# rnajena/dynamont

Measured on AMD Instinct MI355X. Metric: signal samples resquiggled/sec, higher is better.
Workload: dtype f64

## Files before the change

dynamont_amd/_native.py:

```python
from __future__ import annotations

import ctypes as C
import os
import subprocess

HERE = os.path.dirname(os.path.abspath(__file__))
CSRC = os.path.join(HERE, "csrc")
LIB_PATH = os.environ.get("DYN_LIB_PATH") or os.path.join(HERE, "libdynamont_mi.so")
SOURCES = ["dynamont_mi.cpp", "buffers.cpp", "launch.cpp", "session.cpp", "async_engine.cpp", "pore_model.cpp", "csv_format.cpp", "csv_sink.cpp", "vbz_decode.cpp", "bam_reader.cpp", "rccl_comm.cpp", "model_format.cpp",
           "nt_kernels.hip", "pool_stats.hip", "wide_band.hip", "event_stats.hip", "rescale.hip"]
HEADERS = ["engine.hpp", "engine_internal.hpp", "zstd_dl.hpp", "vbz_decode.hpp", "nt_kernels.hpp", "pore_model.hpp", "dp_math.hpp", "dp_math_strict.hpp", "dp_cell.hpp", "strict_exp_table.inc", os.path.join("..", "..", "include", "dynamont_mi.h")]

DYN_DEVICE_HOST_ONLY = -2
DYN_CSV_EVENT_STATS = 0x1
DYN_OK, DYN_ERR_INVALID_ARGUMENT, DYN_ERR_RUNTIME, DYN_ERR_DEVICE, DYN_ERR_OUT_OF_MEMORY = range(5)

c_double_p = C.POINTER(C.c_double)
c_float_p = C.POINTER(C.c_float)
c_u64_p = C.POINTER(C.c_uint64)
c_i32_p = C.POINTER(C.c_int32)
c_u8_p = C.POINTER(C.c_uint8)


class DynInfo(C.Structure):
    _fields_ = [("abi_version", C.c_int32), ("pore", C.c_int32), ("rna", C.c_int32), ("kmer_size", C.c_int32),
                ("alphabet_size", C.c_int32), ("device", C.c_int32), ("num_kmers", C.c_uint64),
                ("half_band", C.c_uint64), ("log_m1", C.c_double), ("log_e1", C.c_double), ("log_e2", C.c_double),
                ("max_half_band", C.c_uint64)]


class DynAlignOut(C.Structure):
    _fields_ = [("Z", c_double_p), ("status", c_i32_p), ("bad_char", C.c_void_p), ("seg_offsets", c_u64_p),
                ("n_segments", c_u64_p), ("sequence_positions", c_u64_p), ("signal_positions", c_u64_p),
                ("probabilities", c_double_p), ("states", c_u8_p), ("capacity", C.c_uint64)]


class DynEventOut(C.Structure):
    _fields_ = [("mean", c_double_p), ("stdev", c_double_p), ("median", c_double_p), ("capacity", C.c_uint64)]


class DynRescaleOut(C.Structure):
    _fields_ = [("shift", c_double_p), ("scale", c_double_p), ("iters_applied", c_i32_p), ("n", C.c_uint64)]


class DynTrainOut(C.Structure):
    _fields_ = [("Z", c_double_p), ("status", c_i32_p), ("bad_char", C.c_void_p), ("transitions", c_double_p),
                ("em_offsets", c_u64_p), ("em_count", c_u64_p), ("em_code", c_i32_p), ("em_mean", c_double_p),
                ("em_stdev", c_double_p), ("em_weight", c_double_p), ("em_sum", c_double_p),
                ("em_sumsq", c_double_p), ("trans_counts", c_double_p), ("capacity", C.c_uint64)]


class DynJobBatch(C.Structure):
    _fields_ = [("n", C.c_uint64),
                ("names", C.c_void_p), ("name_off", C.POINTER(C.c_uint64)), ("names_bytes", C.c_uint64),
                ("signal_ids", C.c_void_p), ("signal_id_off", C.POINTER(C.c_uint64)), ("signal_ids_bytes", C.c_uint64),
                ("signal_uuid", C.c_void_p), ("signal_uuid_ok", C.c_void_p),
                ("seqs", C.c_void_p), ("seq_off", C.POINTER(C.c_uint64)), ("seqs_bytes", C.c_uint64),
                ("shift", C.POINTER(C.c_double)), ("scale", C.POINTER(C.c_double)),
                ("start", C.POINTER(C.c_int64)), ("end", C.POINTER(C.c_int64)),
                ("n_files", C.c_uint64), ("files", C.c_void_p), ("file_off", C.POINTER(C.c_uint64)), ("files_bytes", C.c_uint64),
                ("file_id", C.POINTER(C.c_uint32)), ("bases", C.POINTER(C.c_uint32))]


class DynTiming(C.Structure):
    _fields_ = [("ms_total", C.c_double), ("ms_dp", C.c_double), ("ms_backward", C.c_double), ("ms_forward", C.c_double),
                ("ms_trace", C.c_double), ("wave_wait_share", C.c_double), ("wave_occupancy", C.c_double),
                ("cells", C.c_uint64), ("samples", C.c_uint64), ("reads_ok", C.c_uint64),
                ("launches", C.c_uint32), ("lp_inplace", C.c_uint32), ("pool_pages", C.c_uint32),
                ("page_rows", C.c_uint32), ("n_static", C.c_uint32), ("n_waves", C.c_uint32),
                ("reads_strict", C.c_uint32), ("reserved", C.c_uint32),
                ("ms_backward_strict", C.c_double), ("ms_forward_strict", C.c_double), ("cert_fallbacks", C.c_uint64),
                ("cert_rows", C.c_uint64), ("launch_share", C.c_double)]


class DynSessionStats(C.Structure):
    _fields_ = [("sessions", C.c_uint64), ("tickets", C.c_uint64), ("reads", C.c_uint64), ("cells", C.c_uint64), ("ms", C.c_double),
                ("wave_cycles_busy", C.c_uint64), ("wave_cycles_idle", C.c_uint64), ("wave_cycles_life", C.c_uint64),
                ("waves", C.c_uint64), ("aborted", C.c_uint64), ("republished", C.c_uint64)]


SIGNATURES = {
    "dyn_pore_from_string": (C.c_int, [C.c_char_p, C.POINTER(C.c_int), C.c_char_p, C.c_uint64]),
    "dyn_aligner_create": (C.c_int, [C.c_char_p, C.c_int, C.c_char_p, C.c_int, C.c_uint64, C.c_int,
                                     C.POINTER(C.c_void_p), C.c_char_p, C.c_uint64]),
    "dyn_aligner_destroy": (None, [C.c_void_p]),
    "dyn_release_cached_memory": (None, []),
    "dyn_aligner_set_model": (C.c_int, [C.c_void_p, c_double_p]),
    "dyn_format_model": (C.c_uint64, [C.c_char_p, C.c_int, c_double_p, c_double_p, C.c_uint64, C.c_char_p, C.c_uint64]),
    "dyn_aligner_info": (C.c_int, [C.c_void_p, C.POINTER(DynInfo)]),
    "dyn_aligner_model": (C.c_int, [C.c_void_p, c_double_p]),
    "dyn_aligner_session_stats": (C.c_int, [C.c_void_p, C.POINTER(DynSessionStats)]),
    "dyn_aligner_session_page_wait": (C.c_int, [C.c_void_p, c_u64_p]),
    "dyn_aligner_session_idle_split": (C.c_int, [C.c_void_p, C.POINTER(C.c_uint64)]),
    "dyn_aligner_set_session_mode": (C.c_int, [C.c_void_p, C.c_int, C.c_int]),
    "dyn_aligner_set_mem_budget": (C.c_int, [C.c_void_p, C.c_uint64]),
    "dyn_aligner_set_strict": (C.c_int, [C.c_void_p, C.c_int]),
    "dyn_aligner_set_train_zcheck": (C.c_int, [C.c_void_p, C.c_int]),
    "dyn_aligner_set_event_stats": (C.c_int, [C.c_void_p, C.c_int]),
    "dyn_aligner_set_rescale": (C.c_int, [C.c_void_p, C.c_int]),
    "dyn_tie_rows": (C.c_uint32, [C.c_void_p, c_i32_p, C.c_uint64, C.c_uint64]),
    "dyn_aligner_last_error": (C.c_char_p, [C.c_void_p]),
    "dyn_read_strerror": (C.c_int, [C.c_int, C.c_char, C.c_char_p, C.c_uint64]),
    "dyn_segment_capacity": (C.c_uint64, [C.c_void_p, C.c_uint64, c_u64_p]),
    "dyn_validate_batch": (C.c_int, [C.c_void_p, C.c_uint64, c_u64_p, C.c_char_p, c_u64_p, c_i32_p, C.c_void_p,
                                     c_i32_p, C.c_uint64]),
    "dyn_align_batch": (C.c_int, [C.c_void_p, C.c_uint64, c_double_p, c_u64_p, C.c_char_p, c_u64_p, C.c_int,
                                  C.POINTER(DynAlignOut)]),
    "dyn_train_batch": (C.c_int, [C.c_void_p, C.c_uint64, c_double_p, c_u64_p, C.c_char_p, c_u64_p,
                                  C.POINTER(DynTrainOut), c_double_p]),
    "dyn_format_csv_bound": (C.c_uint64, [C.c_void_p, C.c_uint64, C.POINTER(DynAlignOut), C.POINTER(C.c_char_p),
                                          C.POINTER(C.c_char_p)]),
    "dyn_format_csv": (C.c_int, [C.c_void_p, C.c_uint64, C.POINTER(DynAlignOut), C.c_char_p, c_u64_p,
                                 C.POINTER(C.c_char_p), C.POINTER(C.c_char_p), C.POINTER(C.c_int64),
                                 C.POINTER(C.c_int64), C.c_int, C.c_void_p, C.c_uint64, c_u64_p, c_u64_p]),
    "dyn_format_csv_bound_events": (C.c_uint64, [C.c_void_p, C.c_uint64, C.POINTER(DynAlignOut), C.POINTER(DynEventOut),
                                                 C.POINTER(C.c_char_p), C.POINTER(C.c_char_p)]),
    "dyn_format_csv_events": (C.c_int, [C.c_void_p, C.c_uint64, C.POINTER(DynAlignOut), C.POINTER(DynEventOut), C.c_char_p,
                                        c_u64_p, C.POINTER(C.c_char_p), C.POINTER(C.c_char_p), C.POINTER(C.c_int64),
                                        C.POINTER(C.c_int64), C.c_int, C.c_void_p, C.c_uint64, c_u64_p, c_u64_p]),
    "dyn_csv_compact": (C.c_uint64, [C.c_void_p, C.c_uint64, c_u64_p, c_u64_p]),
    "dyn_csv_sink_open": (C.c_int, [C.c_char_p, C.c_char_p, C.c_int, C.c_int, C.POINTER(C.c_void_p), C.c_char_p, C.c_uint64]),
    "dyn_csv_sink_open_part": (C.c_int, [C.c_char_p, C.c_char_p, C.c_int, C.c_int, C.c_int, C.c_int, C.POINTER(C.c_void_p), C.c_char_p, C.c_uint64]),
    "dyn_csv_sink_open_ex": (C.c_int, [C.c_char_p, C.c_char_p, C.c_int, C.c_int, C.c_int, C.c_int, C.c_uint32,
                                       C.POINTER(C.c_void_p), C.c_char_p, C.c_uint64]),
    "dyn_csv_sink_submit": (C.c_int, [C.c_void_p, C.c_void_p, C.c_void_p, C.POINTER(DynAlignOut), C.c_uint64, C.c_char_p, c_u64_p,
                                      C.POINTER(C.c_char_p), C.POINTER(C.c_char_p), C.POINTER(C.c_int64), c_u64_p]),
    "dyn_csv_sink_submit_bases": (C.c_int, [C.c_void_p, C.c_void_p, C.c_void_p, C.POINTER(DynAlignOut), C.c_uint64, C.c_char_p, c_u64_p,
                                            C.POINTER(C.c_char_p), C.POINTER(C.c_char_p), C.POINTER(C.c_int64), c_u64_p, C.POINTER(C.c_uint32)]),
    "dyn_csv_sink_error_line": (C.c_int, [C.c_void_p, C.c_char_p]),
    "dyn_csv_sink_completed": (C.c_uint64, [C.c_void_p]),
    "dyn_csv_sink_wait": (C.c_uint64, [C.c_void_p, C.c_uint64, C.c_int]),
    "dyn_csv_sink_failed": (C.c_int, [C.c_void_p]),
    "dyn_csv_sink_close": (C.c_int, [C.c_void_p, c_u64_p, c_u64_p, c_u64_p, C.c_char_p, C.c_uint64]),
    "dyn_bam_open": (C.c_int, [C.c_char_p, C.c_int, C.c_char_p, C.POINTER(C.c_void_p), C.c_char_p, C.c_uint64]),
    "dyn_bam_next": (C.c_int, [C.c_void_p, C.c_uint64, C.c_uint32, C.c_double, C.c_uint32, C.c_uint32, C.POINTER(DynJobBatch),
                               C.c_char_p, C.c_uint64]),
    "dyn_bam_skipped": (C.c_uint64, [C.c_void_p]),
    "dyn_bam_close": (None, [C.c_void_p]),
    "dyn_batch_create": (C.c_int, [C.c_void_p, C.c_uint64, c_double_p, c_u64_p, C.c_char_p, c_u64_p,
                                   C.POINTER(C.c_void_p)]),
    "dyn_batch_create_raw": (C.c_int, [C.c_void_p, C.c_uint64, C.c_void_p, C.c_int, c_u64_p, c_double_p, c_double_p,
                                       C.c_int, C.c_double, C.c_int, C.c_char_p, c_u64_p, C.POINTER(C.c_void_p)]),
    "dyn_batch_signals": (C.c_int, [C.c_void_p, c_double_p, C.c_uint64]),
    "dyn_batch_destroy": (None, [C.c_void_p]),
    "dyn_batch_align": (C.c_int, [C.c_void_p, C.c_int]),
    "dyn_batch_train": (C.c_int, [C.c_void_p]),
    "dyn_batch_fetch": (C.c_int, [C.c_void_p, C.POINTER(DynAlignOut)]),
    "dyn_batch_fetch_events": (C.c_int, [C.c_void_p, C.POINTER(DynEventOut)]),
    "dyn_batch_fetch_rescale": (C.c_int, [C.c_void_p, C.POINTER(DynRescaleOut)]),
    "dyn_batch_fetch_train": (C.c_int, [C.c_void_p, C.POINTER(DynTrainOut), c_double_p]),
    "dyn_batch_device_results": (C.c_int, [C.c_void_p, C.POINTER(C.c_void_p), c_u64_p, C.POINTER(C.c_void_p)]),
    "dyn_batch_device_pooled": (C.c_int, [C.c_void_p, C.POINTER(C.c_void_p), c_u64_p]),
    "dyn_batch_timing": (C.c_int, [C.c_void_p, C.POINTER(DynTiming)]),
    "dyn_plan_queue": (C.c_int, [C.c_uint64, C.POINTER(C.c_uint32), c_u64_p, C.c_uint64, C.c_uint64, C.POINTER(C.c_uint32),
                                 c_u64_p, c_u64_p]),
    "dyn_session_order": (C.c_int, [C.c_uint64, C.POINTER(C.c_uint32)]),
    "dyn_batch_align_async": (C.c_int, [C.c_void_p, C.c_uint64, c_double_p, c_u64_p, C.c_char_p, c_u64_p, C.c_int,
                                        C.POINTER(DynAlignOut), C.POINTER(C.c_void_p)]),
    "dyn_batch_train_async": (C.c_int, [C.c_void_p, C.c_uint64, c_double_p, c_u64_p, C.c_char_p, c_u64_p,
                                        C.POINTER(DynTrainOut), c_double_p, C.POINTER(C.c_void_p)]),
    "dyn_batch_align_raw_async": (C.c_int, [C.c_void_p, C.c_uint64, C.c_void_p, C.c_int, c_u64_p, c_float_p, c_float_p, c_double_p, c_double_p,
                                            C.c_int, C.c_double, C.c_int, C.c_char_p, c_u64_p, C.c_int,
                                            C.POINTER(DynAlignOut), C.POINTER(C.c_void_p)]),
    "dyn_batch_train_raw_async": (C.c_int, [C.c_void_p, C.c_uint64, C.c_void_p, C.c_int, c_u64_p, c_float_p, c_float_p, c_double_p, c_double_p,
                                            C.c_int, C.c_double, C.c_int, C.c_char_p, c_u64_p,
                                            C.POINTER(DynTrainOut), c_double_p, C.POINTER(C.c_void_p)]),
    "dyn_batch_align_vbz_async": (C.c_int, [C.c_void_p, C.c_uint64, C.c_void_p, c_u64_p, C.POINTER(C.c_uint32), c_u64_p, c_u64_p, c_u64_p,
                                            c_float_p, c_float_p, c_double_p, c_double_p, C.c_int, C.c_double, C.c_int, C.c_char_p,
                                            c_u64_p, C.c_int, C.POINTER(DynAlignOut), C.POINTER(C.c_void_p)]),
    "dyn_vbz_decode": (C.c_int, [C.c_void_p, C.c_uint64, C.c_uint32, C.c_void_p, C.c_char_p, C.c_uint64]),
    "dyn_batch_wait": (C.c_int, [C.c_void_p]),
    "dyn_host_alloc": (C.c_void_p, [C.c_uint64]),
    "dyn_host_free": (None, [C.c_void_p]),
    "dyn_comm_unique_id": (C.c_int, [c_u8_p, C.c_char_p, C.c_uint64]),
    "dyn_comm_create": (C.c_int, [c_u8_p, C.c_int, C.c_int, C.c_int, C.POINTER(C.c_void_p), C.c_char_p, C.c_uint64]),
    "dyn_comm_destroy": (None, [C.c_void_p]),
    "dyn_comm_last_error": (C.c_char_p, [C.c_void_p]),
    "dyn_comm_gather_counts": (C.c_int, [C.c_void_p, C.c_void_p, c_u64_p]),
    "dyn_comm_gather_rows": (C.c_int, [C.c_void_p, C.c_void_p, C.c_int, C.c_void_p, C.c_uint64, c_u64_p]),
    "dyn_comm_allreduce_pooled": (C.c_int, [C.c_void_p, C.c_void_p, c_double_p]),
    "dyn_comm_gather_bytes": (C.c_int, [C.c_void_p, C.c_void_p, C.c_uint64, C.c_int, c_u64_p]),
    "dyn_comm_gathered_bytes": (C.c_int, [C.c_void_p, C.c_void_p, C.c_uint64]),
    "dyn_comm_allreduce_f64": (C.c_int, [C.c_void_p, c_double_p, C.c_uint64, C.c_int]),
    "dyn_multi_create": (C.c_int, [C.c_char_p, C.c_int, C.c_char_p, C.c_int, C.c_uint64, C.POINTER(C.c_int), C.c_int,
                                   C.POINTER(C.c_void_p), C.c_char_p, C.c_uint64]),
    "dyn_multi_destroy": (None, [C.c_void_p]),
    "dyn_multi_device_count": (C.c_int, [C.c_void_p]),
    "dyn_multi_handle": (C.c_void_p, [C.c_void_p, C.c_int]),
    "dyn_multi_last_error": (C.c_char_p, [C.c_void_p]),
    "dyn_multi_align_batch": (C.c_int, [C.c_void_p, C.c_uint64, c_double_p, c_u64_p, C.c_char_p, c_u64_p, C.c_int,
                                        C.POINTER(DynAlignOut)]),
    "dyn_multi_train_batch": (C.c_int, [C.c_void_p, C.c_uint64, c_double_p, c_u64_p, C.c_char_p, c_u64_p,
                                        C.POINTER(DynTrainOut), c_double_p]),
}


def hipcc_path() -> str:
    for p in (os.environ.get("HIPCC"), "/opt/rocm/bin/hipcc", "hipcc"):
        if p and (os.path.sep not in p or os.path.exists(p)):
            return p
    return "hipcc"


def hipcc_flags() -> list:
    flags = ["--offload-arch=gfx950", "-O3", "-std=c++17", "-fPIC", "-ffp-contract=off", "-Wno-unused-result", "-pthread"]
    return flags + os.environ.get("DYN_HIPCC_EXTRA", "").split()


def needs_build() -> bool:
    if not os.path.exists(LIB_PATH):
        return True
    t = os.path.getmtime(LIB_PATH)
    deps = [os.path.join(CSRC, s) for s in SOURCES + HEADERS]
    return any(os.path.exists(d) and os.path.getmtime(d) > t for d in deps)


def build(force: bool = False, verbose: bool = False) -> str:
    if os.environ.get("DYN_LIB_PATH") or (not force and not needs_build()):
        return LIB_PATH
    import hashlib
    from concurrent.futures import ThreadPoolExecutor
    flags = hipcc_flags()
    objdir = os.path.join(os.path.dirname(HERE), "build", "obj", hashlib.sha1(" ".join(flags).encode()).hexdigest()[:12])
    os.makedirs(objdir, exist_ok=True)
    newest_header = max(os.path.getmtime(os.path.join(CSRC, h)) for h in HEADERS if os.path.exists(os.path.join(CSRC, h)))

    def compile_one(src):
        obj = os.path.join(objdir, src + ".o")
        path = os.path.join(CSRC, src)
        if not force and os.path.exists(obj) and os.path.getmtime(obj) > max(os.path.getmtime(path), newest_header):
            return obj
        cmd = [hipcc_path()] + flags + ["-x", "hip", "-c", path, "-o", obj + ".tmp"]
        if verbose:
            print(" ".join(cmd), flush=True)
        subprocess.run(cmd, check=True)
        os.replace(obj + ".tmp", obj)
        return obj

    with ThreadPoolExecutor(max_workers=min(6, os.cpu_count() or 1)) as ex:
        objs = list(ex.map(compile_one, SOURCES))
    cmd = [hipcc_path(), "--offload-arch=gfx950", "-shared", "-fPIC", "-pthread", "-o", LIB_PATH + ".tmp"] + objs + ["-ldl", "-lz"]
    if verbose:
        print(" ".join(cmd), flush=True)
    subprocess.run(cmd, check=True)
    os.replace(LIB_PATH + ".tmp", LIB_PATH)
    return LIB_PATH


_lib = None


def lib() -> C.CDLL:
    global _lib
    if _lib is None:
        if not os.path.exists(LIB_PATH):
            raise ImportError(
                f"{LIB_PATH} is missing: build it with `python -c 'import __graft_entry__ as g; g.build()'` "
                "(hipcc --offload-arch=gfx950). dynamont_amd has no CPU or PyTorch fallback.")
        import sys
        if "torch" not in sys.modules and int(os.environ.get("WORLD_SIZE", "1") or 1) > 1:
            import torch
        L = C.CDLL(LIB_PATH)
        for name, (res, args) in SIGNATURES.items():
            fn = getattr(L, name)
            fn.restype = res
            fn.argtypes = args
        _lib = L
    return _lib
```

dynamont_amd/csrc/nt_kernels.hip:

```cpp
#include "nt_kernels.hpp"

#include <algorithm>

#include "dp_cell.hpp"
#include "dp_math_strict.hpp"

#define DYN_ONE_WAVE_PER_SIMD \
  __launch_bounds__(256 * DYN_WAVES_PER_SIMD) __attribute__((amdgpu_waves_per_eu(DYN_WAVES_PER_SIMD, DYN_WAVES_PER_SIMD)))

#define DYN_WAVES_PER_GROUP (4 * DYN_WAVES_PER_SIMD)

namespace dynk {

using dynmath::NEG_INF;
using dynmath::EmisV;
using dynmath::log_normal_pdf_vec;
using dynmath::SoftplusNode;
using dynmath::SoftplusLookup;
using dynmath::log_plus_issue;
using dynmath::log_plus_finish;
using dynmath::SP_NODES;

namespace {

typedef __attribute__((address_space(3))) uint32_t lds_u32_t;
typedef __attribute__((address_space(3))) uint64_t lds_u64_t;

__device__ __forceinline__ int pmod(int a) {
  int r = a % P;
  return r < 0 ? r + P : r;
}

__device__ __forceinline__ int pos_of(int lane, int j) { return j < 6 ? (j >> 1) * 128 + lane * 2 + (j & 1) : 384 + lane; }
__device__ __forceinline__ int row_pos(int s) { return pos_of(s / CPL, s % CPL); }

typedef double dyn_d2 __attribute__((ext_vector_type(2)));
typedef float dyn_f2 __attribute__((ext_vector_type(2)));
typedef float dyn_f4 __attribute__((ext_vector_type(4)));

template <bool NT>
__device__ __forceinline__ void store_row_f64(double* __restrict__ row, int lane, const double (&x)[CPL]) {
  static_assert(CPL == 7, "three register pairs and a single");
#pragma unroll
  for (int q = 0; q < 3; ++q) {
    dyn_d2 v;
    v.x = x[2 * q];
    v.y = x[2 * q + 1];
    dyn_d2* dst = reinterpret_cast<dyn_d2*>(row + q * 128 + lane * 2);
    if (NT) __builtin_nontemporal_store(v, dst);
    else *dst = v;
  }
  if (NT) __builtin_nontemporal_store(x[6], row + 384 + lane);
  else row[384 + lane] = x[6];
}

__device__ __forceinline__ uint64_t lanes_of_window(int c0, int len) {
  const int s0 = pmod(c0);
  const int l0 = s0 / CPL;
  const int n = (s0 + len - 1) / CPL - l0 + 1;
  if (n >= 64) return ~0ull;
  const uint64_t m = (1ull << n) - 1ull;
  return l0 ? ((m << l0) | (m >> (64 - l0))) : m;
}
__device__ __forceinline__ uint64_t uniform_u64(uint64_t v) {
  const uint32_t lo32 = (uint32_t)__builtin_amdgcn_readfirstlane((int)(uint32_t)v);
  const uint32_t hi32 = (uint32_t)__builtin_amdgcn_readfirstlane((int)(uint32_t)(v >> 32));
  return ((uint64_t)hi32 << 32) | lo32;
}
__device__ __forceinline__ uint64_t half_mask_of(uint64_t live) {
  uint64_t x = (live | (live >> 1)) & 0x5555555555555555ull;
  x = (x | (x >> 1)) & 0x3333333333333333ull;
  x = (x | (x >> 2)) & 0x0f0f0f0f0f0f0f0full;
  x = (x | (x >> 4)) & 0x00ff00ff00ff00ffull;
  x = (x | (x >> 8)) & 0x0000ffff0000ffffull;
  x = (x | (x >> 16)) & 0x00000000ffffffffull;
  return x;
}
#ifdef DYN_SKIP_OOB
constexpr bool SKIP_OOB = true;
#else
constexpr bool SKIP_OOB = false;
#endif
constexpr int OOB_SLACK = 5;

__device__ __forceinline__ int band_mid(int t, double ratio) {
  return (int)__dmul_rn((double)t, ratio);
}

__device__ __forceinline__ double readlane_f64(double v, int l) {
  int lo = __builtin_amdgcn_readlane(__double2loint(v), l);
  int hi = __builtin_amdgcn_readlane(__double2hiint(v), l);
  return __hiloint2double(hi, lo);
}

__device__ __forceinline__ double wave_ror1(double x) {
  int lo = __double2loint(x), hi = __double2hiint(x);
  const int rlo = __builtin_amdgcn_mov_dpp(lo, 0x13C, 0xf, 0xf, false);
  const int rhi = __builtin_amdgcn_mov_dpp(hi, 0x13C, 0xf, 0xf, false);
  return __hiloint2double(rhi, rlo);
}

__device__ __forceinline__ double wave_rol1(double x) {
  int lo = __double2loint(x), hi = __double2hiint(x);
  const int rlo = __builtin_amdgcn_mov_dpp(lo, 0x134, 0xf, 0xf, false);
  const int rhi = __builtin_amdgcn_mov_dpp(hi, 0x134, 0xf, 0xf, false);
  return __hiloint2double(rhi, rlo);
}

__device__ __forceinline__ void from_left(const double (&x)[CPL], double (&out)[CPL]) {
  out[0] = wave_ror1(x[CPL - 1]);
#pragma unroll
  for (int j = 1; j < CPL; ++j) out[j] = x[j - 1];
}

__device__ __forceinline__ void from_right(const double (&x)[CPL], double (&out)[CPL]) {
#pragma unroll
  for (int j = 0; j < CPL - 1; ++j) out[j] = x[j + 1];
  out[CPL - 1] = wave_rol1(x[0]);
}

__device__ __forceinline__ Emis load_emis(const Emis* __restrict__ pr, int n, int N) {
  Emis e;
  if (n >= 1 && n < N) {
    e = pr[n - 1];
  } else {
    e.mean = 0.0;
    e.inv_stdev = 1.0;
    e.neg_log_stdev = NEG_INF;
    e.stdev = 1.0;
  }
  return e;
}

struct WaveCtx {
  int lane;
  lds_u32_t* pt;
  int log_r;
};

struct RowCursor {
  int page = -1;
  uint32_t base = 0;
  __device__ __forceinline__ uint32_t at(const WaveCtx& w, int t) {
    const int pg = t >> w.log_r;
    if (pg != page) {
      page = pg;
      base = (uint32_t)__builtin_amdgcn_readfirstlane((int)w.pt[pg]) << w.log_r;
    }
    return base + ((uint32_t)t & ((1u << w.log_r) - 1u));
  }
};

__device__ __forceinline__ uint32_t pool_row(const WaveCtx& w, int t) {
  return (w.pt[t >> w.log_r] << w.log_r) + ((uint32_t)t & ((1u << w.log_r) - 1u));
}

__device__ __forceinline__ void wave_lds_sync() {
  __builtin_amdgcn_fence(__ATOMIC_ACQ_REL, "workgroup");
  __builtin_amdgcn_wave_barrier();
}
__device__ __forceinline__ void wave_lds_sync_local() {
  __builtin_amdgcn_fence(__ATOMIC_ACQ_REL, "workgroup", "local");
  __builtin_amdgcn_wave_barrier();
}

constexpr int RING_D = DYN_WAVES_PER_SIMD == 1 ? 4 : 2;
constexpr int ROW_BYTES = P * 8;
constexpr int RING_WAIT = 4 * (RING_D - 1);

#define DYN_DMA_MOD " nt"
__device__ __forceinline__ void ring_dma_row(const double* row_lane_ptr, unsigned lds_slot_addr) {
  asm volatile(
      "s_mov_b32 m0, %1\n\t"
      "s_nop 0\n\t"
      "global_load_lds_dwordx4 %0, off" DYN_DMA_MOD "\n\t"
      "global_load_lds_dwordx4 %0, off offset:1024" DYN_DMA_MOD "\n\t"
      "global_load_lds_dwordx4 %0, off offset:2048" DYN_DMA_MOD "\n\t"
      "s_mov_b32 exec_hi, 0\n\t"
      "global_load_lds_dwordx4 %0, off offset:3072" DYN_DMA_MOD "\n\t"
      "s_mov_b32 exec_hi, -1\n\t"
      ::"v"(row_lane_ptr), "s"(__builtin_amdgcn_readfirstlane(lds_slot_addr))
      : "memory");
}

__device__ __forceinline__ void ring_dma_row_masked(const double* row_lane_ptr, unsigned lds_slot_addr, uint64_t live, uint64_t half) {
  asm volatile(
      "s_mov_b32 m0, %1\n\t"
      "s_mov_b64 exec, %2\n\t"
      "global_load_lds_dwordx4 %0, off" DYN_DMA_MOD "\n\t"
      "global_load_lds_dwordx4 %0, off offset:1024" DYN_DMA_MOD "\n\t"
      "global_load_lds_dwordx4 %0, off offset:2048" DYN_DMA_MOD "\n\t"
      "s_mov_b64 exec, %3\n\t"
      "global_load_lds_dwordx4 %0, off offset:3072" DYN_DMA_MOD "\n\t"
      "s_mov_b64 exec, -1\n\t"
      ::"v"(row_lane_ptr), "s"(__builtin_amdgcn_readfirstlane(lds_slot_addr)), "s"(live), "s"(half)
      : "memory");
}

template <int N>
__device__ __forceinline__ void wait_vmcnt() {
  asm volatile("s_waitcnt vmcnt(%0)" ::"n"(N) : "memory");
}

__device__ __forceinline__ void ring_read_row(unsigned slot_addr, int lane, double (&b)[CPL]) {
  static_assert(CPL == 7, "ring_read_row is written for 7 cells per lane");
  dyn_d2 p0, p1, p2;
  double last;
  asm volatile(
      "ds_read_b128 %0, %4\n\t"
      "ds_read_b128 %1, %4 offset:1024\n\t"
      "ds_read_b128 %2, %4 offset:2048\n\t"
      "ds_read_b64 %3, %5 offset:3072\n\t"
      "s_waitcnt lgkmcnt(0)"
      : "=&v"(p0), "=&v"(p1), "=&v"(p2), "=&v"(last)
      : "v"(slot_addr + lane * 16), "v"(slot_addr + lane * 8)
      : "memory");
  b[0] = p0.x;
  b[1] = p0.y;
  b[2] = p1.x;
  b[3] = p1.y;
  b[4] = p2.x;
  b[5] = p2.y;
  b[6] = last;
}

template <bool STORE, int ARITH>
__device__ __forceinline__ double backward_sweep(const ReadDesc& rd, const WaveCtx& w,
                                                 const double* __restrict__ sig,
                                                 const Emis* __restrict__ par, double* __restrict__ ws,
                                                 double m1, double e2, const SoftplusNode* s_tab, uint32_t* fallbacks = nullptr) {
  const int lane = w.lane;
  uint32_t nfb = 0;
  const int T = (int)rd.T, N = (int)rd.N, bw = (int)rd.bw, W = 2 * bw + 1;
  const double ratio = rd.ratio;
  const double* __restrict__ sg = sig + rd.sig_off;
  const Emis* __restrict__ pr = par + rd.par_off;
  double* __restrict__ out = ws;
  RowCursor cur;

  bool bad_sample = false;
  int lo = band_mid(T - 1, ratio) - bw;
  constexpr bool MASKED = SKIP_OOB && STORE && ARITH != ARITH_FOLDED;
  uint64_t store_mask = MASKED ? uniform_u64(lanes_of_window(lo - OOB_SLACK, W + 2 * OOB_SLACK)) : ~0ull;
  const int n_init = lo + bw;
  int n[CPL];
  double bE[CPL], bM[CPL], bE2[CPL], bM2[CPL], e[CPL];
  EmisV<CPL> p;
  double p_stdev[ARITH == ARITH_STRICT ? CPL : 1];
  double p_ylo[ARITH == ARITH_STRICT ? CPL : 1];
  auto set_p = [&](int j, const Emis& em) {
    set_emis<ARITH>(p, j, em);
    if constexpr (ARITH == ARITH_STRICT) {
      p_stdev[j] = em.stdev;
      p_ylo[j] = dynmath::recip_lo(em.stdev, em.inv_stdev);
    }
  };
  constexpr double SAMPLE_MAX = ARITH == ARITH_STRICT ? 1e300 : 1.7976931348623157e308;
  {
    const size_t rT = STORE ? (size_t)cur.at(w, T) * P : 0, rT1 = STORE ? (size_t)cur.at(w, T - 1) * P : 0;
#pragma unroll
    for (int j = 0; j < CPL; ++j) {
      const int slot = lane * CPL + j;
      n[j] = lo + pmod(slot - lo);
      set_p(j, load_emis(pr, n[j], (n[j] <= lo + W - 1) ? N : 0));
      bE[j] = (n[j] == n_init) ? 0.0 : NEG_INF;
      bM[j] = NEG_INF;
    }
    if (STORE) {
      store_row_f64<false>(out + rT1, lane, bE);
      store_row_f64<false>(out + rT, lane, bM);
    }
  }

  for (int thi = T - 2; thi >= 0; thi -= 64) {
    const int base = thi - 63;
    const int idx = base + lane;
    const double xs = (idx >= 0) ? sg[idx] : 0.0;
    bad_sample |= !(fabs(xs) <= SAMPLE_MAX);
    const int ilo = base < 0 ? -base : 0;
    emission_vec<ARITH>(readlane_f64(xs, 63), p, p_stdev, p_ylo, e);
    auto row = [&](int i, const double (&bE_in)[CPL], const double (&bM_in)[CPL], double (&bE_out)[CPL], double (&bM_out)[CPL]) {
      const int t = base + i;
      double Y[CPL], Yr[CPL], x1[CPL], x2[CPL];
#pragma unroll
      for (int j = 0; j < CPL; ++j) Y[j] = bM_in[j] + e[j];
#pragma unroll
      for (int j = 0; j < CPL; ++j) bM_out[j] = bE_in[j] + e[j];
      from_right(Y, Yr);
      const int new_lo = band_mid(t, ratio) - bw;
      if (__builtin_expect(new_lo != lo, 0)) {
        const int leaving = lo + P - 1;
        const int top = lo + W - 1;
        const Emis fresh = load_emis(pr, new_lo, N);
        const Emis none = load_emis(pr, 0, 0);
#pragma unroll
        for (int j = 0; j < CPL; ++j) {
          if (n[j] == leaving) {
            n[j] = new_lo;
            set_p(j, fresh);
          }
          if (n[j] == top) {
            bM_out[j] = NEG_INF;
            set_p(j, none);
          }
        }
        lo = new_lo;
        if constexpr (MASKED) store_mask = uniform_u64(lanes_of_window(lo - OOB_SLACK, W + 2 * OOB_SLACK));
      }
#pragma unroll
      for (int j = 0; j < CPL; ++j) x1[j] = Yr[j] + m1;
#pragma unroll
      for (int j = 0; j < CPL; ++j) x2[j] = bM_out[j] + e2;
      SoftplusLookup<CPL> L;
      log_plus_issue<CPL>(x1, x2, L, s_tab);
      {
        const double xnext = readlane_f64(xs, i > 0 ? i - 1 : 0);
        emission_vec<ARITH>(xnext, p, p_stdev, p_ylo, e);
      }
      if constexpr (ARITH == ARITH_FOLDED) dynmath::log_plus_finish3<CPL>(L, bE_out);
      else if constexpr (ARITH == ARITH_STRICT) log_plus_finish_certified(L, bE_out, strict_tab(s_tab), nfb);
      else log_plus_finish<CPL>(L, bE_out);
      const size_t rt = STORE ? (size_t)cur.at(w, t) * P : 0;
      if constexpr (STORE && ARITH == ARITH_FOLDED) {
        double ls[CPL];
#pragma unroll
        for (int j = 0; j < CPL; ++j) ls[j] = x2[j] - bE_out[j];
        store_row_f64<true>(out + rt, lane, ls);
      } else if (STORE) {
        if constexpr (MASKED) {
          if (__builtin_amdgcn_inverse_ballot_w64(store_mask)) store_row_f64<true>(out + rt, lane, bE_out);
        } else {
          store_row_f64<true>(out + rt, lane, bE_out);
        }
      }
    };
    int i = 63;
#pragma unroll 1
    for (; i - 1 >= ilo; i -= 2) {
      row(i, bE, bM, bE2, bM2);
      row(i - 1, bE2, bM2, bE, bM);
    }
    if (i >= ilo) {
      row(i, bE, bM, bE2, bM2);
#pragma unroll
      for (int j = 0; j < CPL; ++j) {
        bE[j] = bE2[j];
        bM[j] = bM2[j];
      }
    }
  }
  const bool any_bad = __any(bad_sample);
  if (ARITH == ARITH_STRICT && fallbacks) *fallbacks += nfb;
  return any_bad ? NEG_INF : readlane_f64(bE[0], 0);
}

__device__ __forceinline__ double max_f64(double a, double b) {
  double r;
  asm("v_max_f64 %0, %1, %2" : "=v"(r) : "v"(a), "v"(b));
  return r;
}

template <bool POST, bool INPLACE, bool STRICT>
__device__ __forceinline__ double forward_sweep(const ReadDesc& rd, const WaveCtx& w,
                                                const double* __restrict__ sig, const Emis* __restrict__ par,
                                                const double* __restrict__ ws_rd, float* __restrict__ lp_out,
                                                uint64_t* __restrict__ bits, double Z, double m1, double e2,
                                                const SoftplusNode* s_tab, unsigned ring_base, int strict_rows = 0,
                                                uint32_t* fallbacks = nullptr) {
  uint32_t nfb = 0;
  const int lane = w.lane;
  const int T = (int)rd.T, N = (int)rd.N, bw = (int)rd.bw, W = 2 * bw + 1;
  const double ratio = rd.ratio;
  const double* __restrict__ sg = sig + rd.sig_off;
  const Emis* __restrict__ pr = par + rd.par_off;
  const double* __restrict__ lat = ws_rd;
  float* __restrict__ lat_lp = lp_out;
  RowCursor cur_dma, cur_out;

  int lo = band_mid(1, ratio) - bw;
  constexpr bool MASKED = SKIP_OOB && POST;
  uint64_t dma_mask = ~0ull, dma_half = 0xffffffffull, out_mask = ~0ull;
  auto set_masks = [&]() {
    if constexpr (MASKED) {
      dma_mask = uniform_u64(lanes_of_window(lo, W + OOB_SLACK));
      dma_half = half_mask_of(dma_mask);
      out_mask = uniform_u64(lanes_of_window(lo - 1, W + 1));
    }
  };
  set_masks();
  if constexpr (MASKED) {
    auto* ringp = (__attribute__((address_space(3))) double*)(size_t)ring_base;
#pragma unroll
    for (int k = 0; k < RING_D * P / 64; ++k) ringp[k * 64 + lane] = NEG_INF;
    wave_lds_sync_local();
  }
  int n[CPL];
  struct RowState {
    double fM[CPL], fE[CPL], e[CPL], vM[CPL], vE[CPL], b[CPL];
  };
  RowState sa, sb;
  EmisV<CPL> p;
  double p_stdev[STRICT ? CPL : 1];
  double p_ylo[STRICT ? CPL : 1];
  auto set_p = [&](int j, const Emis& e, auto with_stdev) {
    if constexpr (!POST) set_emis<ARITH_FOLDED>(p, j, e);
    else p.set(j, e);
    if constexpr (STRICT && decltype(with_stdev)::value) {
      p_stdev[j] = e.stdev;
      p_ylo[j] = dynmath::recip_lo(e.stdev, e.inv_stdev);
    }
  };
  auto emission = [&](bool strict_row, double x, double (&out)[CPL]) {
    if constexpr (STRICT) {
      if (strict_row) {
#ifdef DYN_QUOT5
        dynmath::log_normal_pdf_cert_vec<CPL>(x, p, p_stdev, out);
#else
        dynmath::log_normal_pdf_cert4_vec<CPL>(x, p, p_stdev, p_ylo, out);
#endif
        return;
      }
    }
    if constexpr (!POST) emission_vec<ARITH_FOLDED>(x, p, p_stdev, p_ylo, out);
    else log_normal_pdf_vec<CPL>(x, p, out);
  };
  const double x0 = sg[0];
  const size_t r1 = POST ? (size_t)cur_out.at(w, 1) * P : 0;
#pragma unroll
  for (int j = 0; j < CPL; ++j) {
    const int slot = lane * CPL + j;
    n[j] = lo + pmod(slot - lo);
    set_p(j, load_emis(pr, n[j], (n[j] <= lo + W - 1) ? N : 0), std::true_type{});
    sa.fE[j] = (n[j] == 0) ? 0.0 : NEG_INF;
    sa.fM[j] = NEG_INF;
    sa.vE[j] = sa.fE[j];
    sa.vM[j] = NEG_INF;
    sa.b[j] = POST ? lat[r1 + pos_of(lane, j)] : NEG_INF;
  }
  emission(1 <= strict_rows, x0, sa.e);
  const double* __restrict__ dma_src = ws_rd + lane * 2;
  if (POST) {
    for (int r = 2; r <= RING_D + 1; ++r) {
      if constexpr (MASKED) ring_dma_row_masked(dma_src + (size_t)cur_dma.at(w, min(r, T)) * P, ring_base + (r % RING_D) * ROW_BYTES, dma_mask, dma_half);
      else ring_dma_row(dma_src + (size_t)cur_dma.at(w, min(r, T)) * P, ring_base + (r % RING_D) * ROW_BYTES);
    }
  }

  auto row = [&](auto check_move, auto strict_tag, int t, double xn, const RowState& in, RowState& out) {
    constexpr bool STRICT_ROW = STRICT && decltype(strict_tag)::value;
    double fEl[CPL], vEl[CPL];
    if (POST) {
      wait_vmcnt<RING_WAIT>();
      ring_read_row(ring_base + ((t + 1) % RING_D) * ROW_BYTES, lane, out.b);
      if constexpr (MASKED)
        ring_dma_row_masked(dma_src + (size_t)cur_dma.at(w, min(t + 1 + RING_D, T)) * P, ring_base + ((t + 1) % RING_D) * ROW_BYTES, dma_mask, dma_half);
      else
        ring_dma_row(dma_src + (size_t)cur_dma.at(w, min(t + 1 + RING_D, T)) * P, ring_base + ((t + 1) % RING_D) * ROW_BYTES);
    }
    from_left(in.fE, fEl);
    if (POST) from_left(in.vE, vEl);
    if constexpr (decltype(check_move)::value) {
      const int next_lo = band_mid(t + 1, ratio) - bw;
      if (__builtin_expect(next_lo != lo, 0)) {
        const Emis none = load_emis(pr, 0, 0);
        const Emis entering = load_emis(pr, lo + W, N);
#pragma unroll
        for (int j = 0; j < CPL; ++j) {
          const bool leaves = n[j] == lo;
          n[j] = leaves ? lo + P : n[j];
          if (leaves) set_p(j, none, strict_tag);
          if (n[j] == lo + W) set_p(j, entering, strict_tag);
        }
        lo = next_lo;
        set_masks();
      }
    }
    double a1[CPL], a2[CPL];
#pragma unroll
    for (int j = 0; j < CPL; ++j) out.fM[j] = (fEl[j] + in.e[j]) + m1;
#pragma unroll
    for (int j = 0; j < CPL; ++j) a1[j] = in.fM[j] + in.e[j];
#pragma unroll
    for (int j = 0; j < CPL; ++j) a2[j] = (in.fE[j] + in.e[j]) + e2;
    if constexpr (STRICT_ROW) {
      SoftplusLookup<CPL> L;
      log_plus_issue<CPL>(a1, a2, L, s_tab);
      emission(true, xn, out.e);
      log_plus_finish_certified(L, out.fE, strict_tab(s_tab), nfb);
    } else {
      SoftplusLookup<CPL> L;
      log_plus_issue<CPL>(a1, a2, L, s_tab);
      emission(false, xn, out.e);
      if constexpr (!POST) dynmath::log_plus_finish3<CPL>(L, out.fE);
      else log_plus_finish<CPL>(L, out.fE);
    }
    if (POST) {
      double LPM[CPL], LPE[CPL], alt[CPL];
      uint64_t bj[CPL];
#pragma unroll
      for (int j = 0; j < CPL; ++j) LPM[j] = (out.fM[j] + (out.b[j] + out.e[j])) - Z;
#pragma unroll
      for (int j = 0; j < CPL; ++j) LPE[j] = (out.fE[j] + in.b[j]) - Z;
#pragma unroll
      for (int j = 0; j < CPL; ++j) out.vM[j] = vEl[j] + LPM[j];
#pragma unroll
      for (int j = 0; j < CPL; ++j) out.vE[j] = max_f64(in.vM[j], in.vE[j]) + LPE[j];
#pragma unroll
      for (int j = 0; j < CPL; ++j) alt[j] = in.vM[j] + LPE[j];
#pragma unroll
      for (int j = 0; j < CPL; ++j) bj[j] = __ballot(out.vE[j] == alt[j]);
      unsigned wlo, whi;
      static_assert(CPL == 7, "one v_writelane pair per cell register");
#define DYN_WL(J, LO, HI) "v_writelane_b32 %0, %" #LO ", " #J "\n\tv_writelane_b32 %1, %" #HI ", " #J "\n\t"
      asm("s_nop 4\n\t"
          DYN_WL(0, 2, 3) DYN_WL(1, 4, 5) DYN_WL(2, 6, 7) DYN_WL(3, 8, 9) DYN_WL(4, 10, 11) DYN_WL(5, 12, 13) DYN_WL(6, 14, 15)
          : "=&v"(wlo), "=&v"(whi)
          : "s"((unsigned)bj[0]), "s"((unsigned)(bj[0] >> 32)), "s"((unsigned)bj[1]), "s"((unsigned)(bj[1] >> 32)),
            "s"((unsigned)bj[2]), "s"((unsigned)(bj[2] >> 32)), "s"((unsigned)bj[3]), "s"((unsigned)(bj[3] >> 32)),
            "s"((unsigned)bj[4]), "s"((unsigned)(bj[4] >> 32)), "s"((unsigned)bj[5]), "s"((unsigned)(bj[5] >> 32)),
            "s"((unsigned)bj[6]), "s"((unsigned)(bj[6] >> 32)));
#undef DYN_WL
      const uint64_t mybits = ((uint64_t)whi << 32) | wlo;
      const uint32_t prow = cur_out.at(w, t);
      const size_t rt = (size_t)prow * P;
      const bool out_live = MASKED ? __builtin_amdgcn_inverse_ballot_w64(out_mask) : true;
      if (!out_live) {
      } else if (INPLACE) {
#pragma unroll
        for (int q = 0; q < 3; ++q) {
          dyn_f4 v4;
          v4.x = (float)LPM[2 * q];
          v4.y = (float)LPE[2 * q];
          v4.z = (float)LPM[2 * q + 1];
          v4.w = (float)LPE[2 * q + 1];
          __builtin_nontemporal_store(v4, reinterpret_cast<dyn_f4*>(&lat_lp[2 * (rt + q * 128 + lane * 2)]));
        }
        dyn_f2 v2;
        v2.x = (float)LPM[6];
        v2.y = (float)LPE[6];
        __builtin_nontemporal_store(v2, reinterpret_cast<dyn_f2*>(&lat_lp[2 * (rt + 384 + lane)]));
      } else {
#pragma unroll
        for (int q = 0; q < 3; ++q) {
          dyn_f2 v2;
          v2.x = (float)LPE[2 * q];
          v2.y = (float)LPE[2 * q + 1];
          __builtin_nontemporal_store(v2, reinterpret_cast<dyn_f2*>(&lat_lp[rt + q * 128 + lane * 2]));
        }
        __builtin_nontemporal_store((float)LPE[6], &lat_lp[rt + 384 + lane]);
      }
      if (lane < CPL) bits[(size_t)prow * CPL + lane] = mybits;
    }
  };

  auto block = [&](auto strict_tag, int tb) {
    const int idx = tb + lane;
    const double xs = (idx < T - 1) ? sg[idx] : 0.0;
    asm volatile("" ::"v"(xs));
    const int iend = min(64, T - tb);
    int i = 0;
#pragma unroll 1
    for (; i + 1 < iend; i += 2) {
      row(std::true_type{}, strict_tag, tb + i, readlane_f64(xs, i), sa, sb);
      row(std::true_type{}, strict_tag, tb + i + 1, readlane_f64(xs, i + 1), sb, sa);
    }
    if (i < iend) {
      row(std::true_type{}, strict_tag, tb + i, readlane_f64(xs, i), sa, sb);
      sa = sb;
    }
  };
  int tb = 1;
  if constexpr (STRICT) {
    for (; tb < T && tb <= strict_rows; tb += 64) block(std::true_type{}, tb);
  }
  for (; tb < T; tb += 64) block(std::false_type{}, tb);
  const double (&fE)[CPL] = sa.fE;
  if (STRICT && fallbacks) *fallbacks += nfb;
  if (POST) wait_vmcnt<0>();
  const int nf = band_mid(T - 1, ratio);
  const int sf = pmod(nf);
  double zf = 0.0;
#pragma unroll
  for (int j = 0; j < CPL; ++j)
    if (j == sf % CPL) zf = fE[j];
  return readlane_f64(zf, sf / CPL);
}

__device__ __forceinline__ bool z_ok(const ReadDesc& rd, double Zf, double Zb) {
  const double size = (double)((uint64_t)rd.T * (uint64_t)(2 * rd.bw + 3));
  if (isinf(Zf) || isinf(Zb)) return false;
  return !(fabs(Zf - Zb) / size > 1e-8);
}

__device__ __forceinline__ bool traceback(const ReadDesc& rd, const WaveCtx& w, const float* __restrict__ lp,
                                          const uint64_t* __restrict__ bits, TraceBuffers tb, bool inplace,
                                          lds_u64_t* sb) {
  const int lane = w.lane;
  const int T = (int)rd.T, N = (int)rd.N;
  double* __restrict__ pp = tb.pp + rd.path_off;
  uint32_t* __restrict__ pathn = tb.pathn + rd.path_off;
  uint32_t* __restrict__ segrow = tb.segrow + rd.seg_off;

  int t = T - 1, n = N - 1;
  int slot = n % P;
  int stM = 0;
#ifndef DYN_EXP_TB_SERIAL
  uint64_t nb[CPL];
  uint32_t nprow = 0;
  auto fetch = [&](int base_) {
    const int row_ = base_ + lane;
    nprow = 0;
#pragma unroll
    for (int j = 0; j < CPL; ++j) nb[j] = 0;
    if (row_ >= 1) {
      nprow = pool_row(w, row_);
#pragma unroll
      for (int j = 0; j < CPL; ++j) nb[j] = bits[(size_t)nprow * CPL + j];
    }
  };
  int pend_row = 0, pend_n = 0, pend_st = -1;
  float pend_lp = 0.0f;
  auto finish = [&]() {
    if (pend_st >= 0) {
      if (inplace || pend_st == 0) pp[pend_row] = exp((double)pend_lp);
      pathn[pend_row] = (uint32_t)pend_n | (pend_st ? 0x80000000u : 0u);
      if (pend_st) segrow[pend_n - 1] = (uint32_t)pend_row;
    }
    pend_st = -1;
  };
  int sj = slot % CPL, sq = slot / CPL;
  if (t > 0 && n > 0) fetch(t - 63);
  while (t > 0 && n > 0) {
    const int base = t - 63;
    const int row = base + lane;
    const uint32_t prow = nprow;
#pragma unroll
    for (int j = 0; j < CPL; ++j) sb[lane * CPL + j] = nb[j];
    wave_lds_sync_local();
    if (base > 1) fetch(base - 64);
    int my_n = 0, my_st = -1;
    const int block_lo = base < 1 ? 1 : base;
    const uint64_t in_block = base >= 1 ? ~0ull : (~0ull << (1 - base));
    while (t >= block_lo && n > 0) {
      const int tl = t - base;
      if (stM) {
        if (__builtin_amdgcn_inverse_ballot_w64(1ull << tl)) {
          my_n = n;
          my_st = 1;
        }
        --n;
        if (sj == 0) {
          sj = CPL - 1;
          sq = sq ? sq - 1 : 63;
        } else {
          --sj;
        }
        stM = 0;
        --t;
        continue;
      }
      const uint64_t wd = sb[lane * CPL + sj];
      const uint64_t upto = (2ull << tl) - 1ull;
      const uint64_t m = __ballot((wd >> sq) & 1) & upto & in_block;
      if (m) {
        const int rl = 63 - __builtin_clzll(m);
        if (__builtin_amdgcn_inverse_ballot_w64(upto & ~((1ull << rl) - 1ull))) {
          my_n = n;
          my_st = 0;
        }
        if (base + rl - 1 >= block_lo) {
          if (__builtin_amdgcn_inverse_ballot_w64(1ull << (rl - 1))) {
            my_n = n;
            my_st = 1;
          }
          --n;
          if (sj == 0) {
            sj = CPL - 1;
            sq = sq ? sq - 1 : 63;
          } else {
            --sj;
          }
          t = base + rl - 2;
        } else {
          t = base + rl - 1;
          stM = 1;
        }
      } else {
        if (__builtin_amdgcn_inverse_ballot_w64(upto & in_block)) {
          my_n = n;
          my_st = 0;
        }
        t = block_lo - 1;
      }
    }
    finish();
    if (my_st >= 0) {
      const size_t cell = (size_t)prow * P + row_pos(my_n % P);
      if (inplace) pend_lp = lp[2 * cell + (my_st ? 0 : 1)];
      else if (my_st == 0) pend_lp = lp[cell];
      pend_row = row;
      pend_n = my_n;
      pend_st = my_st;
    }
    wave_lds_sync_local();
  }
  finish();
#else
  while (t > 0 && n > 0) {
    const int base = t - 63;
    const int row = base + lane;
    uint32_t prow = 0;
    if (row >= 1) {
      prow = pool_row(w, row);
#pragma unroll
      for (int j = 0; j < CPL; ++j) sb[lane * CPL + j] = bits[(size_t)prow * CPL + j];
    }
    wave_lds_sync();
    int my_n = 0, my_slot = 0, my_st = -1;
    const int block_lo = base < 1 ? 1 : base;
    while (t >= block_lo && n > 0) {
      if (stM) {
        if (row == t) {
          my_n = n;
          my_slot = slot;
          my_st = 1;
        }
        --n;
        slot = slot ? slot - 1 : P - 1;
        stM = 0;
        --t;
        continue;
      }
      const uint64_t wd = sb[lane * CPL + (slot % CPL)];
      const bool bit = (row >= block_lo) && (row <= t) && ((wd >> (slot / CPL)) & 1);
      const uint64_t m = __ballot(bit);
      const int r = m ? base + (63 - __builtin_clzll(m)) : block_lo - 1;
      const int e_lo = m ? r : block_lo;
      if (row >= e_lo && row <= t) {
        my_n = n;
        my_slot = slot;
        my_st = 0;
      }
      if (m) {
        t = r - 1;
        stM = 1;
      } else {
        t = block_lo - 1;
      }
    }
    if (my_st >= 0) {
      const size_t cell = (size_t)prow * P + row_pos(my_slot);
      if (inplace) pp[row] = exp((double)lp[2 * cell + (my_st ? 0 : 1)]);
      else if (my_st == 0) pp[row] = exp((double)lp[cell]);
      pathn[row] = (uint32_t)my_n | (my_st ? 0x80000000u : 0u);
      if (my_st) segrow[my_n - 1] = (uint32_t)row;
    }
    wave_lds_sync();
  }
#endif
  return t == 0 && n == 0;
}

__device__ __forceinline__ void mpost(const ReadDesc& rd, const WaveCtx& w, const double* __restrict__ bE,
                                      const float* __restrict__ lp, const double* __restrict__ sig,
                                      const Emis* __restrict__ par, TraceBuffers tb, double Zb, double m1) {
  const int T = (int)rd.T, N = (int)rd.N;
  const double* __restrict__ sg = sig + rd.sig_off;
  for (int n = 1 + w.lane; n < N; n += 64) {
    const int row = (int)tb.segrow[rd.seg_off + n - 1];
    const int slot = n % P, pslot = (n - 1) % P;
    double fE_prev;
    if (row == 1) {
      fE_prev = n == 1 ? 0.0 : NEG_INF;
    } else {
      const size_t pcell = (size_t)pool_row(w, row - 1) * P + row_pos(pslot);
      fE_prev = ((double)lp[pcell] - bE[pcell]) + Zb;
    }
    const Emis em = par[rd.par_off + n - 1];
    const double e_here = dynmath::log_normal_pdf(sg[row - 1], em);
    const double e_next = row + 1 < T ? dynmath::log_normal_pdf(sg[row], em) : NEG_INF;
    const double fM = (fE_prev + e_here) + m1;
    const double bM = bE[(size_t)pool_row(w, row + 1) * P + row_pos(slot)] + e_next;
    tb.pp[rd.path_off + row] = exp((fM + bM) - Zb);
  }
}

__device__ __forceinline__ double forward_train_chain(const ReadDesc& rd, const WaveCtx& w, const double* __restrict__ sig,
                                                      const double* __restrict__ ws, TrainBuffers tb, double Zb,
                                                      const SoftplusNode* s_tab, unsigned ring_base) {
  const int lane = w.lane;
  const int T = (int)rd.T, N = (int)rd.N, bw = (int)rd.bw;
  const double ratio = rd.ratio;
  const double* __restrict__ sg = sig + rd.sig_off;
  double* __restrict__ cw = tb.col_w + rd.par_off;
  double* __restrict__ cs1 = tb.col_s1 + rd.par_off;
  double* __restrict__ cs2 = tb.col_s2 + rd.par_off;
  const double* __restrict__ etab = exp128_tab(s_tab);
  RowCursor cur_dma;

  int lo = band_mid(1, ratio) - bw;
  double gE[CPL], gM[CPL];
  double aw[CPL], a1[CPL], a2[CPL];
  double awsum = 0.0;
#pragma unroll
  for (int j = 0; j < CPL; ++j) {
    const int nj = lo + pmod(lane * CPL + j - lo);
    gE[j] = (nj == 0) ? 1.0 : 0.0;
    gM[j] = 0.0;
    aw[j] = a1[j] = a2[j] = 0.0;
  }
  const double* __restrict__ dma_src = ws + lane * 2;
  for (int r = 0; r < RING_D; ++r)
    ring_dma_row(dma_src + (size_t)cur_dma.at(w, min(r, T)) * P, ring_base + (r % RING_D) * ROW_BYTES);

  const double one = dynmath::vreg_const(1.0);
  auto row = [&](int t, double x) {
    double ls[CPL], sp[CPL], st[CPL], mv[CPL], mvl[CPL];
    wait_vmcnt<RING_WAIT>();
    const unsigned slot_addr = ring_base + ((t - 1) % RING_D) * ROW_BYTES;
    ring_read_row(slot_addr, lane, ls);
    ring_dma_row(dma_src + (size_t)cur_dma.at(w, min(t - 1 + RING_D, T)) * P, slot_addr);
    dynmath::exp_table128_vec<CPL>(ls, sp, etab);
#pragma unroll
    for (int j = 0; j < CPL; ++j) sp[j] = dynmath::min_hw(sp[j], one);
#pragma unroll
    for (int j = 0; j < CPL; ++j) st[j] = gE[j] * sp[j];
#pragma unroll
    for (int j = 0; j < CPL; ++j) mv[j] = gE[j] - st[j];
    from_left(mv, mvl);
#pragma unroll
    for (int j = 0; j < CPL; ++j) gE[j] = gM[j] + st[j];
    const double x2 = x * x;
#pragma unroll
    for (int j = 0; j < CPL; ++j) {
      gM[j] = mvl[j];
      const double wgt = gE[j] + mvl[j];
      aw[j] += wgt;
      a1[j] = dynmath::fma_(wgt, x, a1[j]);
      a2[j] = dynmath::fma_(wgt, x2, a2[j]);
    }
    const int next_lo = band_mid(t + 1, ratio) - bw;
    if (__builtin_expect(next_lo != lo, 0)) {
#pragma unroll
      for (int j = 0; j < CPL; ++j) {
        const int nj = lo + pmod(lane * CPL + j - lo);
        if (nj == lo - 1 + P) {
          if (lo - 1 >= 1 && lo - 1 < N) {
            cw[lo - 2] = aw[j];
            cs1[lo - 2] = a1[j];
            cs2[lo - 2] = a2[j];
          }
          awsum += aw[j];
          aw[j] = a1[j] = a2[j] = 0.0;
        }
      }
      lo = next_lo;
    }
  };

  for (int tb0 = 1; tb0 < T; tb0 += 64) {
    const int idx = tb0 - 1 + lane;
    const double xs = sg[min(idx, T - 2)];
    asm volatile("" ::"v"(xs));
    const int iend = min(64, T - tb0);
#pragma unroll 1
    for (int i = 0; i < iend; ++i) row(tb0 + i, readlane_f64(xs, i));
  }
  wait_vmcnt<0>();
#pragma unroll
  for (int j = 0; j < CPL; ++j) {
    const int nj = lo + pmod(lane * CPL + j - lo);
// ... 821 lines not shown
```

Before: 531.9.

## Hoist band-shift checks out of DP row loops into run-length segments

Restructures the forward and backward banded DP sweeps so the per-row band_mid computation and band-shift branch are replaced by computing, per run, the last row before the band moves. Rows inside a run execute without the move check, and the emission hand-over happens once at run boundaries. This removes a double multiply, compare and branch from each row's critical path, at the cost of a small search per run and an odd-row tail per run. In the backward sweep, the top-slot reset now writes bE before the row instead of bM_out inside the row, which may or may not be equivalent.

```diff
diff --git a/dynamont_amd/_native.py b/dynamont_amd/_native.py
--- a/dynamont_amd/_native.py
+++ b/dynamont_amd/_native.py
@@ -9,7 +9,7 @@
 LIB_PATH = os.environ.get("DYN_LIB_PATH") or os.path.join(HERE, "libdynamont_mi.so")
 SOURCES = ["dynamont_mi.cpp", "buffers.cpp", "launch.cpp", "session.cpp", "async_engine.cpp", "pore_model.cpp", "csv_format.cpp", "csv_sink.cpp", "vbz_decode.cpp", "bam_reader.cpp", "rccl_comm.cpp", "model_format.cpp",
            "nt_kernels.hip", "pool_stats.hip", "wide_band.hip", "event_stats.hip", "rescale.hip"]
-HEADERS = ["engine.hpp", "engine_internal.hpp", "zstd_dl.hpp", "vbz_decode.hpp", "nt_kernels.hpp", "pore_model.hpp", "dp_math.hpp", "dp_math_strict.hpp", "dp_cell.hpp", "strict_exp_table.inc", os.path.join("..", "..", "include", "dynamont_mi.h")]
+HEADERS = ["engine.hpp", "engine_internal.hpp", "zstd_dl.hpp", "vbz_decode.hpp", "nt_kernels.hpp", "pore_model.hpp", "dp_math.hpp", "dp_math_strict.hpp", "dp_cell.hpp", "band_runs.hpp", "strict_exp_table.inc", os.path.join("..", "..", "include", "dynamont_mi.h")]
 
 DYN_DEVICE_HOST_ONLY = -2
 DYN_CSV_EVENT_STATS = 0x1
diff --git a/dynamont_amd/csrc/band_runs.hpp b/dynamont_amd/csrc/band_runs.hpp
--- /dev/null
+++ b/dynamont_amd/csrc/band_runs.hpp
@@ -0,0 +1,41 @@
+#pragma once
+
+#if defined(__HIPCC__)
+#include <hip/hip_runtime.h>
+#define DYN_BR_HD __host__ __device__ __forceinline__
+#else
+#define DYN_BR_HD inline
+#endif
+
+namespace dynband {
+
+DYN_BR_HD int band_mid(int t, double ratio) {
+#if defined(__HIP_DEVICE_COMPILE__)
+  return (int)__dmul_rn((double)t, ratio);
+#else
+  return (int)((double)t * ratio);
+#endif
+}
+
+DYN_BR_HD int first_row_reaching(int m, double ratio, double inv_ratio, int lo_row, int hi_row) {
+  const double guess = (double)m * inv_ratio;
+  int q = guess < (double)hi_row ? (int)guess : hi_row;
+  if (q < lo_row) q = lo_row;
+  while (band_mid(q, ratio) < m) ++q;
+  while (q > lo_row && band_mid(q - 1, ratio) >= m) --q;
+  return q;
+}
+
+DYN_BR_HD int next_move_row(int t, double ratio, double inv_ratio, int limit) {
+  if (t >= limit) return limit;
+  const int m = band_mid(t, ratio);
+  if (band_mid(limit, ratio) == m) return limit;
+  return first_row_reaching(m + 1, ratio, inv_ratio, t + 1, limit) - 1;
+}
+
+DYN_BR_HD int run_first_row(int t, double ratio, double inv_ratio, int floor_row) {
+  if (t <= floor_row) return t;
+  return first_row_reaching(band_mid(t, ratio), ratio, inv_ratio, floor_row, t);
+}
+
+}
diff --git a/dynamont_amd/csrc/nt_kernels.hip b/dynamont_amd/csrc/nt_kernels.hip
--- a/dynamont_amd/csrc/nt_kernels.hip
+++ b/dynamont_amd/csrc/nt_kernels.hip
@@ -2,6 +2,7 @@
 
 #include <algorithm>
 
+#include "band_runs.hpp"
 #include "dp_cell.hpp"
 #include "dp_math_strict.hpp"
 
@@ -83,9 +84,7 @@
 #endif
 constexpr int OOB_SLACK = 5;
 
-__device__ __forceinline__ int band_mid(int t, double ratio) {
-  return (int)__dmul_rn((double)t, ratio);
-}
+using dynband::band_mid;
 
 __device__ __forceinline__ double readlane_f64(double v, int l) {
   int lo = __builtin_amdgcn_readlane(__double2loint(v), l);
@@ -240,6 +239,7 @@
 
   bool bad_sample = false;
   int lo = band_mid(T - 1, ratio) - bw;
+  const double inv_ratio = 1.0 / ratio;
   constexpr bool MASKED = SKIP_OOB && STORE && ARITH != ARITH_FOLDED;
   uint64_t store_mask = MASKED ? uniform_u64(lanes_of_window(lo - OOB_SLACK, W + 2 * OOB_SLACK)) : ~0ull;
   const int n_init = lo + bw;
@@ -279,34 +279,33 @@
     bad_sample |= !(fabs(xs) <= SAMPLE_MAX);
     const int ilo = base < 0 ? -base : 0;
     emission_vec<ARITH>(readlane_f64(xs, 63), p, p_stdev, p_ylo, e);
-    auto row = [&](int i, const double (&bE_in)[CPL], const double (&bM_in)[CPL], double (&bE_out)[CPL], double (&bM_out)[CPL]) {
-      const int t = base + i;
+    auto hand_over = [&](int new_lo) {
+      const int leaving = lo + P - 1;
+      const int top = lo + W - 1;
+      const Emis fresh = load_emis(pr, new_lo, N);
+      const Emis none = load_emis(pr, 0, 0);
+#pragma unroll
+      for (int j = 0; j < CPL; ++j) {
+        if (n[j] == leaving) {
+          n[j] = new_lo;
+          set_p(j, fresh);
+        }
+        if (n[j] == top) {
+          bE[j] = NEG_INF;
+          set_p(j, none);
+        }
+      }
+      lo = new_lo;
+      if constexpr (MASKED) store_mask = uniform_u64(lanes_of_window(lo - OOB_SLACK, W + 2 * OOB_SLACK));
+    };
+    auto row = [&](int t, const double (&bE_in)[CPL], const double (&bM_in)[CPL], double (&bE_out)[CPL], double (&bM_out)[CPL]) {
+      const int i = t - base;
       double Y[CPL], Yr[CPL], x1[CPL], x2[CPL];
 #pragma unroll
       for (int j = 0; j < CPL; ++j) Y[j] = bM_in[j] + e[j];
 #pragma unroll
       for (int j = 0; j < CPL; ++j) bM_out[j] = bE_in[j] + e[j];
       from_right(Y, Yr);
-      const int new_lo = band_mid(t, ratio) - bw;
-      if (__builtin_expect(new_lo != lo, 0)) {
-        const int leaving = lo + P - 1;
-        const int top = lo + W - 1;
-        const Emis fresh = load_emis(pr, new_lo, N);
-        const Emis none = load_emis(pr, 0, 0);
-#pragma unroll
-        for (int j = 0; j < CPL; ++j) {
-          if (n[j] == leaving) {
-            n[j] = new_lo;
-            set_p(j, fresh);
-          }
-          if (n[j] == top) {
-            bM_out[j] = NEG_INF;
-            set_p(j, none);
-          }
-        }
-        lo = new_lo;
-        if constexpr (MASKED) store_mask = uniform_u64(lanes_of_window(lo - OOB_SLACK, W + 2 * OOB_SLACK));
-      }
 #pragma unroll
       for (int j = 0; j < CPL; ++j) x1[j] = Yr[j] + m1;
 #pragma unroll
@@ -334,18 +333,26 @@
         }
       }
     };
-    int i = 63;
+    int t = thi;
+    const int tlo = base + ilo;
 #pragma unroll 1
-    for (; i - 1 >= ilo; i -= 2) {
-      row(i, bE, bM, bE2, bM2);
-      row(i - 1, bE2, bM2, bE, bM);
-    }
-    if (i >= ilo) {
-      row(i, bE, bM, bE2, bM2);
-#pragma unroll
-      for (int j = 0; j < CPL; ++j) {
-        bE[j] = bE2[j];
-        bM[j] = bM2[j];
+    while (t >= tlo) {
+      const int new_lo = band_mid(t, ratio) - bw;
+      if (new_lo != lo) hand_over(new_lo);
+      const int tq = __builtin_amdgcn_readfirstlane(dynband::run_first_row(t, ratio, inv_ratio, tlo));
+#pragma unroll 1
+      for (; t - 1 >= tq; t -= 2) {
+        row(t, bE, bM, bE2, bM2);
+        row(t - 1, bE2, bM2, bE, bM);
+      }
+      if (t >= tq) {
+        row(t, bE, bM, bE2, bM2);
+#pragma unroll
+        for (int j = 0; j < CPL; ++j) {
+          bE[j] = bE2[j];
+          bM[j] = bM2[j];
+        }
+        --t;
       }
     }
   }
@@ -378,6 +385,7 @@
   RowCursor cur_dma, cur_out;
 
   int lo = band_mid(1, ratio) - bw;
+  const double inv_ratio = 1.0 / ratio;
   constexpr bool MASKED = SKIP_OOB && POST;
   uint64_t dma_mask = ~0ull, dma_half = 0xffffffffull, out_mask = ~0ull;
   auto set_masks = [&]() {
@@ -446,7 +454,21 @@
     }
   }
 
-  auto row = [&](auto check_move, auto strict_tag, int t, double xn, const RowState& in, RowState& out) {
+  auto hand_over = [&](auto strict_tag, int next_lo) {
+    const Emis none = load_emis(pr, 0, 0);
+    const Emis entering = load_emis(pr, lo + W, N);
+#pragma unroll
+    for (int j = 0; j < CPL; ++j) {
+      const bool leaves = n[j] == lo;
+      n[j] = leaves ? lo + P : n[j];
+      if (leaves) set_p(j, none, strict_tag);
+      if (n[j] == lo + W) set_p(j, entering, strict_tag);
+    }
+    lo = next_lo;
+    set_masks();
+  };
+
+  auto row = [&](auto strict_tag, int t, double xn, const RowState& in, RowState& out) {
     constexpr bool STRICT_ROW = STRICT && decltype(strict_tag)::value;
     double fEl[CPL], vEl[CPL];
     if (POST) {
@@ -459,22 +481,6 @@
     }
     from_left(in.fE, fEl);
     if (POST) from_left(in.vE, vEl);
-    if constexpr (decltype(check_move)::value) {
-      const int next_lo = band_mid(t + 1, ratio) - bw;
-      if (__builtin_expect(next_lo != lo, 0)) {
-        const Emis none = load_emis(pr, 0, 0);
-        const Emis entering = load_emis(pr, lo + W, N);
-#pragma unroll
-        for (int j = 0; j < CPL; ++j) {
-          const bool leaves = n[j] == lo;
-          n[j] = leaves ? lo + P : n[j];
-          if (leaves) set_p(j, none, strict_tag);
-          if (n[j] == lo + W) set_p(j, entering, strict_tag);
-        }
-        lo = next_lo;
-        set_masks();
-      }
-    }
     double a1[CPL], a2[CPL];
 #pragma unroll
     for (int j = 0; j < CPL; ++j) out.fM[j] = (fEl[j] + in.e[j]) + m1;
@@ -557,16 +563,23 @@
     const int idx = tb + lane;
     const double xs = (idx < T - 1) ? sg[idx] : 0.0;
     asm volatile("" ::"v"(xs));
-    const int iend = min(64, T - tb);
-    int i = 0;
+    const int tend = tb + min(64, T - tb);
+    int t = tb;
 #pragma unroll 1
-    for (; i + 1 < iend; i += 2) {
-      row(std::true_type{}, strict_tag, tb + i, readlane_f64(xs, i), sa, sb);
-      row(std::true_type{}, strict_tag, tb + i + 1, readlane_f64(xs, i + 1), sb, sa);
-    }
-    if (i < iend) {
-      row(std::true_type{}, strict_tag, tb + i, readlane_f64(xs, i), sa, sb);
-      sa = sb;
+    while (t < tend) {
+      const int next_lo = band_mid(t + 1, ratio) - bw;
+      if (next_lo != lo) hand_over(strict_tag, next_lo);
+      const int te = __builtin_amdgcn_readfirstlane(dynband::next_move_row(t + 1, ratio, inv_ratio, tend));
+#pragma unroll 1
+      for (; t + 1 < te; t += 2) {
+        row(strict_tag, t, readlane_f64(xs, t - tb), sa, sb);
+        row(strict_tag, t + 1, readlane_f64(xs, t + 1 - tb), sb, sa);
+      }
+      if (t < te) {
+        row(strict_tag, t, readlane_f64(xs, t - tb), sa, sb);
+        sa = sb;
+        ++t;
+      }
     }
   };
   int tb = 1;
```

New measurement: 544.7 (median of 6 runs). 2.4% higher.
